# dayae1204/WeCLIP-ViT-CoMer

Hardware: AMD Instinct MI355X
Metric: images/sec (train fwd+bwd) ViT-B/16 512x512 VOC (higher is better)
Workload: dtype f16 MFMA operands / f32 accumulate, f32 residual+softmax+LN, PAR f32 arithmetic on 16-bit fixed-point affinities (precision=fast); 1 GPU; WeCLIP VOC full train step (the reference's model: frozen CLIP ViT-B/16 + adapters + decoder + GradCAM/affinity/PAR pseudo-labels), batch 16/GPU at 512x512, K=2 classes/image (BASELINE configs[2] without the ViT-CoMer inserts, for which the reference has no code); global_batch=16, parallelism=dp1

## Files before the change

include/weclip_hip.h:

```cpp
#ifndef WECLIP_HIP_H
#define WECLIP_HIP_H
#include <stdint.h>
#ifdef __cplusplus
extern "C" {
#endif

int wc_version(void);
const char* wc_last_error(void);
int wc_device_count(void);
int wc_device_arch(int dev, char* buf, int buflen);

void wc_prof_enable(int stride);
void wc_prof_tag(const char* tag);
int wc_prof_report(char* buf, int cap);

int wc_par_affinity(const float* img, float* aff, int B, int H, int W,
                    const int* h_dilations, int n_dil, void* stream);
int wc_par_iterate(const float* aff, const float* masks_in, float* masks_out, int B, int C,
                   int H, int W, const int* h_dilations, int n_dil, void* stream);
int wc_par_forward(const float* img, const float* masks, float* out, float* tmp, float* aff_ws,
                   int B, int C, int H, int W, const int* h_dilations, int n_dil, int num_iter,
                   int group, void* stream);
int wc_par_forward_h(const float* img, const float* masks, float* out, float* tmp, float* aff_ws,
                   int B, int C, int H, int W, const int* h_dilations, int n_dil, int num_iter,
// ... 60 lines not shown
                   int x_rpg, int x_gs, int x_off, int mslice, int bias, float* part, void* stream);
int wc_gemm_km_f16_grouped(const void* dY, long lda, const void* X, long ldx, const void* zeros, int M, int N, int K,
                           int x_rpg, int x_gs, int x_off, int mslice, int bias, float* part, int groups, long gA,
                           long gX, void* stream);
int wc_gemm_km_f16_multi(const int64_t* jobs, int count, const void* zeros, void* stream);
int wc_gemm_km_multi_plan(const int64_t* jobs, int count, int cus, int* launch, int* first, int* pos, int* grids,
                          int* forms, int max_launches, int* nlaunches);
int wc_gemm_km_multi_locate(const int64_t* jobs, int count, int cus, int l, int wg, int* out);
int wc_split_f16(const float* x, void* hi, void* lo, long n, void* stream);

int wc_convert_weights(const int64_t* table, int count, int blocks_per_tensor, void* stream);

int wc_adamw_multi(const int64_t* table, int count, double lr, double beta1, double beta2, double eps,
                   double weight_decay, double bias_correction1, double bias_correction2, int blocks_per_tensor,
                   void* stream);

int wc_sgd_multi(const int64_t* table, int count, double lr, double momentum, double weight_decay, int blocks_per_tensor,
                 void* stream);

int wc_layernorm(const float* x, long ldx, const float* w, const float* b, float eps, float* y32,
                 void* y16, void* y16lo, long rows, int D, void* stream);

int wc_attn_fwd(const void* qkv, void* out, float* out32, float* lse, int B, int L, int H, int DH,
                void* stream);
int wc_attn_mean(const void* qkv, const float* lse, float* mean, int B, int L, int H, int DH,
                 void* stream);

int wc_patchify(const float* img, void* hi, void* lo, int B, int H, int W, int P, void* stream);
int wc_cls_rows(float* x, const float* cls, const float* pos0, int B, int L, int E, void* stream);

int wc_cam_head(const float* x2, const float* lnw, const float* lnb, const float* proj,
                const float* text, const int* text_idx, const int* n_text, const int* pair_img,
                const int* pair_cls, float logit_scale, float* partial, float* probs, float* df,
                int B, int P, int L, int E, int Ed, int Tmax, void* stream);
int wc_lnpost_bwd(const float* df, const float* x2, const float* lnw, float gs, const int* pair_img,
                  float* d32, void* dhi, void* dlo, int P, int L, int E, void* stream);
int wc_ln2_bwd_add(const float* da2, const float* dx2, const float* x1, const float* lnw, float gs,
                   const int* pair_img, void* g16, int P, int L, int E, void* stream);
int wc_attn_bwd_colsum(const void* qkv, const void* dO, const float* o32, const float* lse,
                       const int* pair_img, float* delta, float* u, float* dS0, float* P0, float* c,
                       int P, int L, int H, int DH, void* stream);
int wc_rowvec_matmul(const float* c, const float* W, float* out, float* ws, int P, int N, int E, float scale,
                     void* stream);
int wc_cam_map(const float* a32, const float* w, const int* pair_img, float* cam, int P, int L, int E,
               void* stream);

int wc_aff_weight(const float* const* h_maps, int nmaps, const float* wgt, const float* seg, float* W,
                  int B, int L, void* stream);
int wc_aff_seg_weights(const float* const* h_maps, int nmaps, float* rowsum, float* diff, float* wgt,
                       int B, int L, void* stream);
int wc_matvec(const float* W, const float* X, const float* sin, const float* sout, const float* add,
              float* out, int B, int hw, int K, int transpose, int recip, float alpha, void* stream);
int wc_aff_fused_supported(int hw);
int wc_aff_weight_c1(const float* const* h_maps, int nmaps, const float* wgt, const float* seg, float* W, float* c1,
                     float* ws, int B, int L, void* stream);
int wc_attn_aff_weight(const void* const* h_qkv, const float* const* h_lse, int nmaps, const float* wgt, float* W, float* c1,
                       float* ws, int B, int L, int H, int DH, void* stream);
int wc_aff_sinkhorn_step(const float* W, const float* c, float* r, float* c_next, float* ws, int B, int hw, int last,
                         void* stream);
int wc_aff_tsym_apply(const float* W, const float* r, const float* c, const float* X, float* out, float* y1, float* ws,
                      int B, int hw, int K, void* stream);
int wc_tsym(const float* W, const float* r, const float* c, float* T, int B, int hw, void* stream);
int wc_box_mask(const float* cam, const int* pair_img, const int* pair_slot, float* V, float* mask_out,
                int* boxes, int* nbox, int maxbox, int P, int h, int w, int K, double thr, void* stream);
int wc_cam_upsample(const float* R, const int* nk, float* stats, float* cams, int B, int h, int w, int K,
                    int C, int H, int W, void* stream);

int wc_attn_bwd(const void* qkv, const void* dO, const float* o32, const float* lse, void* qt, void* kt,
                void* dot, float* delta, void* dqkv_hi, void* dqkv_lo, int B, int L, int Lp, int H, int DH,
                void* stream);
int wc_transpose_f16(const void* src, int src_f32, long ld, long sSrc, void* hi, void* lo, long ldo,
                     long oR, int batch, int R, int C, float scale, void* stream);
int wc_colsum(const void* src, int src_f32, long ld, float* part, float* out, long R, int C, float alpha,
              int round16, void* stream);
int wc_layernorm_bwd(const float* dy, const float* x, const float* w, const float* add, float eps,
                     float* dx32, void* dx16, float out_scale, float* part, float* dgb, float alpha,
                     long rows, int D, void* stream);
int wc_layernorm_bwd_h(const void* dy16, const float* x, const float* w, const float* add, float eps,
                       float* dx32, void* dx16, float out_scale, float* part, float* dgb, float alpha,
                       long rows, int D, void* stream);
int wc_layernorm_bwd2_h(const void* dya16, const float* wa, const void* dyb16, const float* wb, const float* x,
                        const float* add, float eps, float* dx32, void* dx16, float out_scale, float* part, float* dgba,
                        float* dgbb, float alpha, long rows, int D, void* stream);
int wc_sigmoid_gram_bwd(const float* dAP, const float* AP, void* hi, void* lo, int B, int n, int ldo,
                        float scale, void* stream);
int wc_colscale_split(const float* x, const float* cs, float* out32, void* hi, void* lo, long rows, int C,
                      int rows_per_batch, float alpha, void* stream);

int wc_msda_fwd(const float* value, const int* h_shapes, int n_levels, const float* loc, const float* attn,
                float* out, int N, int Lq, int M, int D, int P, void* stream);
int wc_msda_fwd_h(const void* value, int value_is_f16, const int* h_shapes, int n_levels, const float* loc,
                  const float* attn, float* out, void* out16, int N, int Lq, int M, int D, int P, void* stream);
int wc_msda_bwd(const float* value, const int* h_shapes, int n_levels, const float* loc, const float* attn,
                const float* gout, float* gvalue, float* gloc, float* gattn, void* gmax, void* ws, int N, int Lq, int M,
                int D, int P, void* stream);
int wc_msda_bwd_h(const void* value, int value_is_f16, const int* h_shapes, int n_levels, const float* loc,
                  const float* attn, const void* gout, int gout_is_f16, float* gvalue, void* gvalue16, float* gloc,
// ... 189 lines not shown
```

weclip-vit-comer_amd/csrc/affinity.hip:

```cpp
#include "common.h"
#include "resample.h"

#define MAXK 4

struct MapPtrs {
    const float* p[12];
};

__global__ __launch_bounds__(256) void aff_weight_kernel(MapPtrs maps, int nmaps, const float* __restrict__ wgt,
                                                          const float* __restrict__ seg, float* __restrict__ W,
                                                          int L) {
    const int hw = L - 1;
    const int j = blockIdx.x * 256 + threadIdx.x, i = blockIdx.y, b = blockIdx.z;
    if (j >= hw) return;
    const long src = (long)b * L * L + (long)(i + 1) * L + (j + 1);
    float v[12];
#pragma unroll
    for (int l = 0; l < 12; ++l) v[l] = l < nmaps ? maps.p[l][src] : 0.f;
    float s = 0.f;
#pragma unroll
    for (int l = 0; l < 12; ++l)
        if (l < nmaps) s = fmaf(wgt[b * nmaps + l], v[l], s);
    const long dst = ((long)b * hw + i) * hw + j;
    if (seg) s *= seg[dst];
// ... 300 lines not shown
    }
}

__global__ __launch_bounds__(256) void aff_colreduce_kernel(const float* __restrict__ colpart, const float* __restrict__ y1,
                                                             const float* __restrict__ c, float* __restrict__ out, int hw,
                                                             int K, int nblk, int mode) {
    const int e = blockIdx.x * 256 + threadIdx.x, b = blockIdx.y;
    if (e >= hw * K) return;
    const float* cp = colpart + (long)b * nblk * hw * K + e;
    const long st = (long)hw * K;
    float s = 0.f;
    int blk = 0;
    for (; blk + 8 <= nblk; blk += 8) {
        float v[8];
#pragma unroll
        for (int u = 0; u < 8; ++u) v[u] = cp[(blk + u) * st];
        s += ((v[0] + v[1]) + (v[2] + v[3])) + ((v[4] + v[5]) + (v[6] + v[7]));
    }
    for (; blk < nblk; ++blk) s += cp[blk * st];
    if (mode == 0) out[(long)b * hw + e] = 1.0f / s;
    else out[(long)b * hw * K + e] = 0.5f * (y1[(long)b * hw * K + e] + c[(long)b * hw + e / K] * s);
}

__global__ __launch_bounds__(256) void tsym_kernel(const float* __restrict__ W, const float* __restrict__ r,
                                                    const float* __restrict__ c, float* __restrict__ T, int hw) {
    const int j = blockIdx.x * 256 + threadIdx.x, i = blockIdx.y, b = blockIdx.z;
    if (j >= hw) return;
    const float* Wb = W + (long)b * hw * hw;
    const float* rb = r + (long)b * hw;
    const float* cb = c + (long)b * hw;
    T[((long)b * hw + i) * hw + j] = 0.5f * (rb[i] * Wb[(long)i * hw + j] * cb[j] + cb[i] * Wb[(long)j * hw + i] * rb[j]);
}

__global__ __launch_bounds__(256) void box_mask_kernel(const float* __restrict__ cam, const int* __restrict__ pair_img,
                                                        const int* __restrict__ pair_slot, float* __restrict__ V,
                                                        float* __restrict__ mask_out, int* __restrict__ boxes,
                                                        int* __restrict__ nbox, int maxbox, int h, int w, int K,
                                                        double thr) {
    extern __shared__ int smi[];
    const int hw = h * w, p = blockIdx.x, tid = threadIdx.x;
    int* lab = smi;
    int* xmin = lab + hw;
    int* xmax = xmin + hw;
    int* ymin = xmax + hw;
    int* ymax = ymin + hw;
    int* roots = ymax + hw;
    int* misc = roots + hw;
    const float* cp = cam + (long)p * hw;
    if (tid == 0) { misc[0] = 0; misc[2] = 0; }
    __syncthreads();
    int mx = 0;
    for (int i = tid; i < hw; i += 256) {
        const int u = (int)(unsigned char)(cp[i] * 255.0f);
        mx = u > mx ? u : mx;
    }
    atomicMax(&misc[0], mx);
    __syncthreads();
    const int theta = (int)(thr * (double)misc[0]);
    for (int i = tid; i < hw; i += 256) {
        const int u = (int)(unsigned char)(cp[i] * 255.0f);
        lab[i] = (u > theta) ? i : -1;
        xmin[i] = w; xmax[i] = -1; ymin[i] = h; ymax[i] = -1;
    }
    __syncthreads();
    for (int it = 0; it < hw + 2; ++it) {
        if (tid == 0) misc[1] = 0;
        __syncthreads();
        int changed = 0;
        for (int i = tid; i < hw; i += 256) {
            int l = lab[i];
            if (l < 0) continue;
// ... 27 lines not shown
        const int y = i / w, x = i - y * w;
        atomicMin(&xmin[l], x); atomicMax(&xmax[l], x);
        atomicMin(&ymin[l], y); atomicMax(&ymax[l], y);
    }
    __syncthreads();
    for (int i = tid; i < hw; i += 256)
        if (lab[i] == i) roots[atomicAdd(&misc[2], 1)] = i;
    __syncthreads();
    const int nroot = misc[2];
    if (boxes) {
        if (tid == 0) nbox[p] = nroot;
        for (int k = tid; k < nroot && k < maxbox; k += 256) {
            const int r = roots[k];
            int* bx = boxes + ((long)p * maxbox + k) * 4;
            bx[0] = xmin[r]; bx[1] = ymin[r];
            bx[2] = (xmax[r] + 1 < w - 1) ? xmax[r] + 1 : w - 1;
            bx[3] = (ymax[r] + 1 < h - 1) ? ymax[r] + 1 : h - 1;
        }
    }
    const int img = pair_img[p], slot = pair_slot[p];
    for (int i = tid; i < hw; i += 256) {
        const int y = i / w, x = i - y * w;
        int inside = 0;
        for (int k = 0; k < nroot && !inside; ++k) {
            const int r = roots[k];
            const int x0 = xmin[r], y0 = ymin[r];
            int x1 = xmax[r] + 1, y1 = ymax[r] + 1;
            x1 = x1 < w - 1 ? x1 : w - 1;
            y1 = y1 < h - 1 ? y1 : h - 1;
            inside = (x >= x0 && x < x1 && y >= y0 && y < y1);
        }
        if (mask_out) mask_out[(long)p * hw + i] = inside ? 1.f : 0.f;
        if (slot >= 0) V[((long)img * hw + i) * K + slot] = inside ? cp[i] : 0.f;
    }
}

__global__ __launch_bounds__(256) void refined_minmax_kernel(const float* __restrict__ R, float* __restrict__ stats,
                                                              int hw, int K) {
    __shared__ float red[16];
    const int k = blockIdx.x, b = blockIdx.y;
    float mn = INFINITY, mx = -INFINITY;
    for (int i = threadIdx.x; i < hw; i += 256) {
        const float v = R[((long)b * hw + i) * K + k];
        mn = fminf(mn, v);
        mx = fmaxf(mx, v);
    }
    mn = block_min(mn, red);
    mx = block_max(mx, red);
    if (threadIdx.x == 0) {
        stats[((long)b * K + k) * 2] = mn;
        stats[((long)b * K + k) * 2 + 1] = mx - mn;
    }
}

__global__ __launch_bounds__(256) void cam_upsample_kernel(const float* __restrict__ R, const float* __restrict__ stats,
                                                            const int* __restrict__ nk, float* __restrict__ cams,
                                                            int h, int w, int K, int C, int H, int W, float sy, float sx) {
    const int x = blockIdx.x * 64 + (threadIdx.x & 63), y = blockIdx.y * 4 + (threadIdx.x >> 6), b = blockIdx.z;
    if (x >= W || y >= H) return;
    int y0, y1, x0, x1;
    float ly, lx;
    wc_bil_src(y, h, sy, y0, y1, ly);
    wc_bil_src(x, w, sx, x0, x1, lx);
    const long HW = (long)H * W;
    const int n = nk[b];
    float best = -INFINITY;
// ... 96 lines not shown
        WC_LAUNCH_CHECK("aff_colreduce_kernel");
    }
    return WC_OK;
}

extern "C" int wc_aff_tsym_apply(const float* W, const float* r, const float* c, const float* X, float* out, float* y1,
                                 float* ws, int B, int hw, int K, void* stream) {
    WC_CHECK_ARG(W && r && c && X && out && y1 && ws && out != X && B > 0 && B <= 65535 && K >= 1 && K <= 4 && aff_fused_ok(hw),
                 "wc_aff_tsym_apply: bad argument (K <= 4)");
    const int nblk = wc_cdiv(hw, AF_RPB);
    hipStream_t st = (hipStream_t)stream;
    dim3 grid(nblk, B);
    const int pr = wc_prof_begin(stream);
    switch (K) {
        case 1: hipLaunchKernelGGL((aff_sweep_kernel<2, 1>), grid, dim3(256), 0, st, W, c, r, X, nullptr, y1, ws, hw); break;
        case 2: hipLaunchKernelGGL((aff_sweep_kernel<2, 2>), grid, dim3(256), 0, st, W, c, r, X, nullptr, y1, ws, hw); break;
        case 3: hipLaunchKernelGGL((aff_sweep_kernel<2, 3>), grid, dim3(256), 0, st, W, c, r, X, nullptr, y1, ws, hw); break;
        default: hipLaunchKernelGGL((aff_sweep_kernel<2, 4>), grid, dim3(256), 0, st, W, c, r, X, nullptr, y1, ws, hw); break;
    }
    wc_prof_end(pr, "aff_sweep_kernel", (double)B * hw * hw * 4.0 * 2, stream);
    WC_LAUNCH_CHECK("aff_sweep_kernel");
    hipLaunchKernelGGL(aff_colreduce_kernel, dim3(wc_cdiv(hw * K, 256), B), dim3(256), 0, st, ws, y1, c, out, hw, K, nblk, 1);
    WC_LAUNCH_CHECK("aff_colreduce_kernel");
    return WC_OK;
}

extern "C" int wc_tsym(const float* W, const float* r, const float* c, float* T, int B, int hw, void* stream) {
    WC_CHECK_ARG(W && r && c && T && B > 0 && hw > 0, "wc_tsym: bad argument");
    hipLaunchKernelGGL(tsym_kernel, dim3(wc_cdiv(hw, 256), hw, B), dim3(256), 0, (hipStream_t)stream, W, r, c, T, hw);
    WC_LAUNCH_CHECK("tsym_kernel");
    return WC_OK;
}

extern "C" int wc_box_mask(const float* cam, const int* pair_img, const int* pair_slot, float* V, float* mask_out,
                           int* boxes, int* nbox, int maxbox, int P, int h, int w, int K, double thr, void* stream) {
    WC_CHECK_ARG(cam && pair_img && pair_slot && V && P > 0 && h > 0 && w > 0 && K > 0, "wc_box_mask: bad argument");
    WC_CHECK_ARG(!boxes || (nbox && maxbox > 0), "wc_box_mask: boxes needs nbox and maxbox");
    const size_t sm = ((size_t)6 * h * w + 4) * sizeof(int);
    WC_CHECK_ARG(sm <= 160 * 1024, "wc_box_mask: CAM grid too large (h*w <= 6800)");
    hipLaunchKernelGGL(box_mask_kernel, dim3(P), dim3(256), sm, (hipStream_t)stream, cam, pair_img, pair_slot, V,
                       mask_out, boxes, nbox, maxbox, h, w, K, thr);
    WC_LAUNCH_CHECK("box_mask_kernel");
    return WC_OK;
}

extern "C" int wc_cam_upsample(const float* R, const int* nk, float* stats, float* cams, int B, int h, int w, int K,
                               int C, int H, int W, void* stream) {
    WC_CHECK_ARG(R && nk && stats && cams && B > 0 && h > 0 && w > 0 && K > 0 && C >= 2 && C <= K + 1 && H > 0 && W > 0,
                 "wc_cam_upsample: bad argument");
    hipStream_t st = (hipStream_t)stream;
    hipLaunchKernelGGL(refined_minmax_kernel, dim3(K, B), dim3(256), 0, st, R, stats, h * w, K);
    WC_LAUNCH_CHECK("refined_minmax_kernel");
    hipLaunchKernelGGL(cam_upsample_kernel, dim3(wc_cdiv(W, 64), wc_cdiv(H, 4), B), dim3(256), 0, st, R, stats, nk,
                       cams, h, w, K, C, H, W, (float)h / H, (float)w / W);
    WC_LAUNCH_CHECK("cam_upsample_kernel");
    return WC_OK;
}
```

weclip-vit-comer_amd/csrc/gradcam.hip:

```cpp
#include "common.h"

typedef _Float16 f16x8 __attribute__((ext_vector_type(8)));
typedef float f32x16 __attribute__((ext_vector_type(16)));

#define LNP_ROWS 16
template <int NV>
__global__ __launch_bounds__(256) void lnpost_pool_kernel(const float* __restrict__ x2,
                                                           const float* __restrict__ w,
                                                           const float* __restrict__ bb, float eps,
                                                           float* __restrict__ partial, int L, int E,
                                                           int nchunk) {
    extern __shared__ float sm[];
    const int b = blockIdx.y, chunk = blockIdx.x, lane = threadIdx.x & 63, wv = threadIdx.x >> 6;
    float acc[NV], wv_[NV], bv[NV];
#pragma unroll
    for (int i = 0; i < NV; ++i) {
        const int e = lane + 64 * i;
        acc[i] = 0.f;
        wv_[i] = e < E ? w[e] : 0.f;
        bv[i] = e < E ? bb[e] : 0.f;
    }
    const int l0 = chunk * LNP_ROWS;
    for (int l = l0 + wv; l < l0 + LNP_ROWS && l < L; l += 4) {
        if (l == 0) continue;
        const float* xr = x2 + ((long)b * L + l) * E;
        float xv[NV];
        float s = 0.f;
#pragma unroll
        for (int i = 0; i < NV; ++i) {
            const int e = lane + 64 * i;
            xv[i] = e < E ? xr[e] : 0.f;
            s += xv[i];
        }
        const float mean = wave_sum(s) / E;
        float q = 0.f;
#pragma unroll
        for (int i = 0; i < NV; ++i) {
            const float d = (lane + 64 * i < E) ? xv[i] - mean : 0.f;
            q += d * d;
        }
        const float rstd = rsqrtf(wave_sum(q) / E + eps);
#pragma unroll
        for (int i = 0; i < NV; ++i)
            if (lane + 64 * i < E) acc[i] += (xv[i] - mean) * rstd * wv_[i] + bv[i];
    }
#pragma unroll
    for (int i = 0; i < NV; ++i)
        if (lane + 64 * i < E) sm[wv * E + lane + 64 * i] = acc[i];
    __syncthreads();
    for (int e = threadIdx.x; e < E; e += 256)
        partial[((long)b * nchunk + chunk) * E + e] = sm[e] + sm[E + e] + sm[2 * E + e] + sm[3 * E + e];
}

__global__ __launch_bounds__(512) void cam_head_kernel(const float* __restrict__ partial,
                                                        const float* __restrict__ proj,
                                                        const float* __restrict__ text,
                                                        const int* __restrict__ text_idx,
                                                        const int* __restrict__ n_text,
                                                        const int* __restrict__ pair_img,
                                                        const int* __restrict__ pair_cls, float logit_scale,
                                                        float* __restrict__ probs, float* __restrict__ df,
                                                        int L, int E, int Ed, int nchunk, int Tmax) {
    extern __shared__ float sm[];
    float* f = sm;
    float* y = f + E;
    float* dy = y + Ed;
    float* lg = dy + Ed;
    float* red = lg + Tmax;
    const int p = blockIdx.x, img = pair_img[p], cls = pair_cls[p], T = n_text[p], tid = threadIdx.x;
    for (int e = tid; e < E; e += 512) {
        const float* pp = partial + (long)img * nchunk * E + e;
        float s[8] = {0.f, 0.f, 0.f, 0.f, 0.f, 0.f, 0.f, 0.f};
        int c = 0;
        for (; c + 8 <= nchunk; c += 8)
#pragma unroll
            for (int u = 0; u < 8; ++u) s[u] += pp[(long)(c + u) * E];
        for (; c < nchunk; ++c) s[0] += pp[(long)c * E];
        f[e] = (((s[0] + s[1]) + (s[2] + s[3])) + ((s[4] + s[5]) + (s[6] + s[7]))) / (L - 1);
    }
    __syncthreads();
    for (int t = tid; t < Ed; t += 512) {
        float s0 = 0.f, s1 = 0.f, s2 = 0.f, s3 = 0.f;
        int e = 0;
        for (; e + 16 <= E; e += 16) {
            float pv[16];
#pragma unroll
            for (int u = 0; u < 16; ++u) pv[u] = proj[(long)(e + u) * Ed + t];
#pragma unroll
            for (int u = 0; u < 16; u += 4) {
                s0 = fmaf(f[e + u], pv[u], s0);
                s1 = fmaf(f[e + u + 1], pv[u + 1], s1);
                s2 = fmaf(f[e + u + 2], pv[u + 2], s2);
                s3 = fmaf(f[e + u + 3], pv[u + 3], s3);
            }
        }
        for (; e < E; ++e) s0 = fmaf(f[e], proj[(long)e * Ed + t], s0);
        y[t] = (s0 + s1) + (s2 + s3);
    }
    __syncthreads();
    float q = 0.f;
    for (int t = tid; t < Ed; t += 512) q += y[t] * y[t];
    const float ynorm = sqrtf(block_sum(q, red));
    __syncthreads();
    for (int t = tid; t < Ed; t += 512) y[t] /= ynorm;
    __syncthreads();
    const int lane = tid & 63, wv = tid >> 6;
    for (int t = wv; t < T; t += 8) {
        const float* tr = text + (long)text_idx[(long)p * Tmax + t] * Ed;
        float s = 0.f;
        for (int k = lane; k < Ed; k += 64) s += y[k] * tr[k];
        s = wave_sum(s);
        if (lane == 0) lg[t] = logit_scale * s;
    }
    __syncthreads();
    float mx = -INFINITY;
    for (int t = 0; t < T; ++t) mx = fmaxf(mx, lg[t]);
    float den = 0.f;
    for (int t = 0; t < T; ++t) den += expf(lg[t] - mx);
    __syncthreads();
    if (tid < T) {
        const float pr = expf(lg[tid] - mx) / den;
        probs[(long)p * Tmax + tid] = pr;
        lg[tid] = pr;
    }
    __syncthreads();
    const float pj = lg[cls];
    for (int k = tid; k < Ed; k += 512) {
        float s = 0.f;
        for (int t = 0; t < T; ++t) {
            const float dl = pj * ((t == cls ? 1.f : 0.f) - lg[t]);
            s = fmaf(dl, text[(long)text_idx[(long)p * Tmax + t] * Ed + k], s);
        }
        dy[k] = logit_scale * s;
    }
    __syncthreads();
    float dot = 0.f;
    for (int k = tid; k < Ed; k += 512) dot += y[k] * dy[k];
    dot = block_sum(dot, red);
    __syncthreads();
    for (int k = tid; k < Ed; k += 512) dy[k] = (dy[k] - y[k] * dot) / ynorm;
    __syncthreads();
    if ((Ed & 3) == 0) {
        const int rsub = lane >> 3, j = lane & 7;
        for (int e0 = wv * 8; e0 < E; e0 += 64) {
            const int e = e0 + rsub;
            float s = 0.f;
            if (e < E) {
                const float* pr = proj + (long)e * Ed;
#pragma unroll 4
                for (int k = 4 * j; k < Ed; k += 32) {
                    const float4 pv = *reinterpret_cast<const float4*>(pr + k);
                    s = fmaf(pv.x, dy[k], s);
                    s = fmaf(pv.y, dy[k + 1], s);
                    s = fmaf(pv.z, dy[k + 2], s);
                    s = fmaf(pv.w, dy[k + 3], s);
                }
            }
            s += __shfl_xor(s, 1, 64);
            s += __shfl_xor(s, 2, 64);
            s += __shfl_xor(s, 4, 64);
            if (j == 0 && e < E) df[(long)p * E + e] = s;
        }
    } else {
        for (int e = tid; e < E; e += 512) {
            const float* pr = proj + (long)e * Ed;
            float s = 0.f;
            for (int k = 0; k < Ed; ++k) s = fmaf(pr[k], dy[k], s);
            df[(long)p * E + e] = s;
        }
    }
}

template <int NV>
__global__ __launch_bounds__(256) void lnpost_bwd_kernel(const float* __restrict__ df,
                                                          const float* __restrict__ x2,
                                                          const float* __restrict__ w, float eps, float gs,
                                                          const int* __restrict__ pair_img,
                                                          float* __restrict__ d32, __half* __restrict__ dhi,
                                                          __half* __restrict__ dlo, int L, int E, long rows) {
    const long row = (long)blockIdx.x * 4 + (threadIdx.x >> 6);
    if (row >= rows) return;
    const int lane = threadIdx.x & 63;
    const int p = row / L, l = row % L;
    const long o = row * E;
    if (l == 0) {
        for (int e = lane; e < E; e += 64) {
            d32[o + e] = 0.f;
            dhi[o + e] = __float2half(0.f);
            if (dlo) dlo[o + e] = __float2half(0.f);
        }
        return;
    }
    const float* xr = x2 + ((long)pair_img[p] * L + l) * E;
    const float* g0 = df + (long)p * E;
    const float invn = 1.0f / (L - 1);
    if constexpr (NV > 0) {
        float xv[NV], gv[NV];
        float s = 0.f;
#pragma unroll
        for (int i = 0; i < NV; ++i) {
            const int e = lane + 64 * i, ec = e < E ? e : 0;
            const float ok = e < E ? 1.f : 0.f;
            xv[i] = xr[ec] * ok;
// ... 405 lines not shown
    const int p = blockIdx.y, img = pair_img[p], lane = threadIdx.x & 63, wv = threadIdx.x >> 6;
    const int l = blockIdx.x * 16 + wv, hw = L - 1;
    if (l >= hw) return;
    const float* ar = a32 + ((long)img * L + l + 1) * E;
    const float* wr = w + (long)p * E;
    float s = 0.f;
    for (int e = lane; e < E; e += 64) s = fmaf(wr[e], ar[e], s);
    s = wave_sum(s);
    if (lane == 0) cam[(long)p * hw + l] = fmaxf(s, 0.f);
}

__global__ __launch_bounds__(1024) void cam_norm_kernel(float* __restrict__ cam, int hw) {
    extern __shared__ float sm[];
    float* cs = sm;
    float* red = cs + hw;
    const int p = blockIdx.x, tid = threadIdx.x;
    for (int l = tid; l < hw; l += 1024) cs[l] = cam[(long)p * hw + l];
    __syncthreads();
#pragma unroll 1
    for (int pass = 0; pass < 2; ++pass) {
        float mn = INFINITY;
        for (int l = tid; l < hw; l += 1024) mn = fminf(mn, cs[l]);
        mn = block_min(mn, red);
        float mx = -INFINITY;
        for (int l = tid; l < hw; l += 1024) mx = fmaxf(mx, cs[l] - mn);
        mx = block_max(mx, red);
        __syncthreads();
        for (int l = tid; l < hw; l += 1024) cs[l] = fmaxf((cs[l] - mn) / (1e-7f + mx), 0.f);
        __syncthreads();
    }
    for (int l = tid; l < hw; l += 1024) cam[(long)p * hw + l] = cs[l];
}

extern "C" int wc_cam_head(const float* x2, const float* lnw, const float* lnb, const float* proj,
                           const float* text, const int* text_idx, const int* n_text, const int* pair_img,
                           const int* pair_cls, float logit_scale, float* partial, float* probs, float* df,
                           int B, int P, int L, int E, int Ed, int Tmax, void* stream) {
    WC_CHECK_ARG(x2 && lnw && lnb && proj && text && text_idx && n_text && pair_img && pair_cls && partial &&
                     probs && df && B > 0 && P > 0 && L > 1 && E > 0 && Ed > 0,
                 "wc_cam_head: bad argument");
    WC_CHECK_ARG(Tmax > 0 && Tmax <= 512 && E <= 4096 && Ed <= 4096, "wc_cam_head: Tmax <= 512, E, Ed <= 4096");
    hipStream_t st = (hipStream_t)stream;
    const int nchunk = wc_cdiv(L, LNP_ROWS);
    WC_CHECK_ARG(E <= 1024, "wc_cam_head: E <= 1024");
    if (E <= 256)
        hipLaunchKernelGGL(lnpost_pool_kernel<4>, dim3(nchunk, B), dim3(256), 4 * E * sizeof(float), st, x2, lnw, lnb,
                           1e-5f, partial, L, E, nchunk);
    else
        hipLaunchKernelGGL(lnpost_pool_kernel<16>, dim3(nchunk, B), dim3(256), 4 * E * sizeof(float), st, x2, lnw, lnb,
                           1e-5f, partial, L, E, nchunk);
    WC_LAUNCH_CHECK("lnpost_pool_kernel");
    const size_t sm = (E + 2 * Ed + Tmax + 16) * sizeof(float);
    hipLaunchKernelGGL(cam_head_kernel, dim3(P), dim3(512), sm, st, partial, proj, text, text_idx, n_text,
                       pair_img, pair_cls, logit_scale, probs, df, L, E, Ed, nchunk, Tmax);
    WC_LAUNCH_CHECK("cam_head_kernel");
    return WC_OK;
}

extern "C" int wc_lnpost_bwd(const float* df, const float* x2, const float* lnw, float gs,
                             const int* pair_img, float* d32, void* dhi, void* dlo, int P, int L, int E,
                             void* stream) {
    WC_CHECK_ARG(df && x2 && lnw && pair_img && d32 && dhi && P > 0 && L > 1 && E > 0,
                 "wc_lnpost_bwd: bad argument");
    const long rows = (long)P * L;
#define LNPOST_BWD(NV_)                                                                                            \
    hipLaunchKernelGGL(lnpost_bwd_kernel<NV_>, dim3(wc_cdiv(rows, 4)), dim3(256), 0, (hipStream_t)stream, df, x2, \
                       lnw, 1e-5f, gs, pair_img, d32, (__half*)dhi, (__half*)dlo, L, E, rows)
    if (E <= 256) LNPOST_BWD(4);
    else if (E <= 768) LNPOST_BWD(12);
    else if (E <= 1024) LNPOST_BWD(16);
    else LNPOST_BWD(0);
#undef LNPOST_BWD
    WC_LAUNCH_CHECK("lnpost_bwd_kernel");
    return WC_OK;
}

extern "C" int wc_ln2_bwd_add(const float* da2, const float* dx2, const float* x1, const float* lnw, float gs,
                              const int* pair_img, void* g16, int P, int L, int E, void* stream) {
    WC_CHECK_ARG(da2 && dx2 && x1 && lnw && pair_img && g16 && P > 0 && L > 0 && E > 0 && gs > 0,
                 "wc_ln2_bwd_add: bad argument");
    const long rows = (long)P * L;
    WC_CHECK_ARG(E <= 1024, "wc_ln2_bwd_add: E <= 1024");
    if (E <= 256)
        hipLaunchKernelGGL(ln2_bwd_add_kernel<4>, dim3(wc_cdiv(rows, 4)), dim3(256), 0, (hipStream_t)stream, da2,
                           dx2, x1, lnw, 1e-5f, 1.0f / gs, pair_img, (__half*)g16, L, E, rows);
    else if (E <= 768)
        hipLaunchKernelGGL(ln2_bwd_add_kernel<12>, dim3(wc_cdiv(rows, 4)), dim3(256), 0, (hipStream_t)stream, da2,
                           dx2, x1, lnw, 1e-5f, 1.0f / gs, pair_img, (__half*)g16, L, E, rows);
    else
// ... 123 lines not shown
```

weclip-vit-comer_amd/gradcam_engine.py:

```python
import torch

from . import _lib as L
from . import ops
from .ops import F16, F32, Split
from .clip import vit_engine as VE

def _logit_scale(clip_model):
    p = clip_model.logit_scale
    key = (p.data_ptr(), p._version)
    cached = getattr(clip_model, "_logit_scale_host", None)
    if cached is None or cached[0] != key:
        cached = (key, float(p.detach().exp().item()))
        clip_model._logit_scale_host = cached
    return cached[1]


GRAD_SCALE = 4096.0


class _BwdPack:

    def __init__(self, blk):
        t = lambda w: ops.split_f16(w.detach().float().t().contiguous())
        self.pjT = t(blk.mlp.c_proj.weight)
        self.fcT = t(blk.mlp.c_fc.weight)
        self.outT = t(blk.attn.out_proj.weight)
        self.w_in = blk.attn.in_proj_weight.detach().float().contiguous()
        self.ln2_w = blk.ln_2.weight.detach().float().contiguous()


class LastLayerState:

    def __init__(self, clip_model, x2, mean, keep, B, Lq):
        self.m, self.x2, self.mean, self.keep, self.B, self.L = clip_model, x2, mean, keep, B, Lq
        blk = clip_model.visual.transformer.resblocks[-1]
        if getattr(blk, "_bwd_pack", None) is None or blk._bwd_pack.w_in.device != x2.device:
            blk._bwd_pack = _BwdPack(blk)
        self.bw = blk._bwd_pack
        self.blk = blk

    def _head(self, text_hat, text_idx, n_text, pair_img, pair_cls, Tmax):
        v = self.m.visual
        B, Lq = self.B, self.L
        E, Ed = v.proj.shape
        P = pair_img.numel()
        dev = self.x2.device
        nchunk = (Lq + 15) // 16
        partial = torch.empty(B * nchunk * E, device=dev, dtype=F32)
        probs = torch.zeros(P, Tmax, device=dev, dtype=F32)
        df = torch.empty(P, E, device=dev, dtype=F32)
        L.lib().wc_cam_head(L.ptr(self.x2, F32), L.ptr(v.ln_post.weight.detach().float(), F32),
                            L.ptr(v.ln_post.bias.detach().float(), F32),
                            L.ptr(v.proj.detach().float().contiguous(), F32), L.ptr(text_hat, F32),
                            L.ptr(text_idx, torch.int32), L.ptr(n_text, torch.int32),
                            L.ptr(pair_img, torch.int32), L.ptr(pair_cls, torch.int32),
                            _logit_scale(self.m), L.ptr(partial), L.ptr(probs),
                            L.ptr(df), B, P, Lq, E, Ed, Tmax, L.stream())
        return probs, df

    def class_probs(self, text):
        dev = self.x2.device
        T = text.shape[0]
        that = (text / text.norm(dim=1, keepdim=True)).contiguous()
        idx = torch.arange(T, dtype=torch.int32, device=dev).repeat(self.B, 1).contiguous()
        nt = torch.full((self.B,), T, dtype=torch.int32, device=dev)
        img = torch.arange(self.B, dtype=torch.int32, device=dev)
        cls = torch.zeros(self.B, dtype=torch.int32, device=dev)
        probs, _ = self._head(that, idx, nt, img, cls, T)
        return probs

    def grad_cam(self, text_hat, text_idx, n_text, pair_img, pair_cls, Tmax):
        lib = L.lib()
        k, bw = self.keep, self.bw
        B, Lq = self.B, self.L
        E = self.x2.shape[1]
        H = self.blk.attn.num_heads
        DH = E // H
        P = pair_img.numel()
        M = P * Lq
        dev = self.x2.device
        st = L.stream
        probs, df = self._head(text_hat, text_idx, n_text, pair_img, pair_cls, Tmax)
        v = self.m.visual
        dx2 = torch.empty(M, E, device=dev, dtype=F32)
        from . import config
        ex = config.exact()
        dx2s = Split(torch.empty(M, E, device=dev, dtype=F16), torch.empty(M, E, device=dev, dtype=F16) if ex else None)
        lib.wc_lnpost_bwd(L.ptr(df), L.ptr(self.x2), L.ptr(v.ln_post.weight.detach().float(), F32),
                          GRAD_SCALE, L.ptr(pair_img), L.ptr(dx2), L.ptr(dx2s.hi), L.ptr(dx2s.lo), P, Lq, E,
                          st())
# ... 29 lines not shown
```

Measured before the change: 1314 images/sec.

## Parallelize CAM head and box-mask kernels across more blocks and threads

The CAM head is split into three kernels: a per-image projection spread over many blocks, a per-pair softmax/gradient kernel, and a df kernel tiled over rows of the projection. This replaces the single block per pair that recomputed the full projection serially. The box-mask connected-component kernel now runs with up to 1024 threads per block instead of 256 and caches each thread's cam value. The old single-block paths remain as _single entry points. These are small pseudo-label stages, so the gain in end-to-end throughput is likely modest, and the split adds launches and intermediate buffers.

```diff
diff --git a/include/weclip_hip.h b/include/weclip_hip.h
--- a/include/weclip_hip.h
+++ b/include/weclip_hip.h
@@ -116,7 +116,11 @@
 int wc_cam_head(const float* x2, const float* lnw, const float* lnb, const float* proj,
                 const float* text, const int* text_idx, const int* n_text, const int* pair_img,
                 const int* pair_cls, float logit_scale, float* partial, float* probs, float* df,
-                int B, int P, int L, int E, int Ed, int Tmax, void* stream);
+                float* y, float* dy, int B, int P, int L, int E, int Ed, int Tmax, void* stream);
+int wc_cam_head_single(const float* x2, const float* lnw, const float* lnb, const float* proj,
+                       const float* text, const int* text_idx, const int* n_text, const int* pair_img,
+                       const int* pair_cls, float logit_scale, float* partial, float* probs, float* df,
+                       float* y, float* dy, int B, int P, int L, int E, int Ed, int Tmax, void* stream);
 int wc_lnpost_bwd(const float* df, const float* x2, const float* lnw, float gs, const int* pair_img,
                   float* d32, void* dhi, void* dlo, int P, int L, int E, void* stream);
 int wc_ln2_bwd_add(const float* da2, const float* dx2, const float* x1, const float* lnw, float gs,
@@ -147,6 +151,8 @@
 int wc_tsym(const float* W, const float* r, const float* c, float* T, int B, int hw, void* stream);
 int wc_box_mask(const float* cam, const int* pair_img, const int* pair_slot, float* V, float* mask_out,
                 int* boxes, int* nbox, int maxbox, int P, int h, int w, int K, double thr, void* stream);
+int wc_box_mask_single(const float* cam, const int* pair_img, const int* pair_slot, float* V, float* mask_out,
+                       int* boxes, int* nbox, int maxbox, int P, int h, int w, int K, double thr, void* stream);
 int wc_cam_upsample(const float* R, const int* nk, float* stats, float* cams, int B, int h, int w, int K,
                     int C, int H, int W, void* stream);
 
diff --git a/weclip-vit-comer_amd/csrc/affinity.hip b/weclip-vit-comer_amd/csrc/affinity.hip
--- a/weclip-vit-comer_amd/csrc/affinity.hip
+++ b/weclip-vit-comer_amd/csrc/affinity.hip
@@ -356,11 +356,11 @@
     T[((long)b * hw + i) * hw + j] = 0.5f * (rb[i] * Wb[(long)i * hw + j] * cb[j] + cb[i] * Wb[(long)j * hw + i] * rb[j]);
 }
 
-__global__ __launch_bounds__(256) void box_mask_kernel(const float* __restrict__ cam, const int* __restrict__ pair_img,
-                                                        const int* __restrict__ pair_slot, float* __restrict__ V,
-                                                        float* __restrict__ mask_out, int* __restrict__ boxes,
-                                                        int* __restrict__ nbox, int maxbox, int h, int w, int K,
-                                                        double thr) {
+__global__ __launch_bounds__(256) void box_mask_single_kernel(const float* __restrict__ cam, const int* __restrict__ pair_img,
+                                                               const int* __restrict__ pair_slot, float* __restrict__ V,
+                                                               float* __restrict__ mask_out, int* __restrict__ boxes,
+                                                               int* __restrict__ nbox, int maxbox, int h, int w, int K,
+                                                               double thr) {
     extern __shared__ int smi[];
     const int hw = h * w, p = blockIdx.x, tid = threadIdx.x;
     int* lab = smi;
@@ -454,6 +454,130 @@
         }
         if (mask_out) mask_out[(long)p * hw + i] = inside ? 1.f : 0.f;
         if (slot >= 0) V[((long)img * hw + i) * K + slot] = inside ? cp[i] : 0.f;
+    }
+}
+
+__global__ __launch_bounds__(1024) void box_mask_kernel(const float* __restrict__ cam, const int* __restrict__ pair_img,
+                                                         const int* __restrict__ pair_slot, float* __restrict__ V,
+                                                         float* __restrict__ mask_out, int* __restrict__ boxes,
+                                                         int* __restrict__ nbox, int maxbox, int h, int w, int K,
+                                                         double thr) {
+    extern __shared__ int smi[];
+    const int hw = h * w, p = blockIdx.x, tid = threadIdx.x, nthr = blockDim.x;
+    int* lab = smi;
+    int* xmin = lab + hw;
+    int* xmax = xmin + hw;
+    int* ymin = xmax + hw;
+    int* ymax = ymin + hw;
+    int* roots = ymax + hw;
+    int* misc = roots + hw;
+    const float* cp = cam + (long)p * hw;
+    const float c0 = tid < hw ? cp[tid] : 0.f;
+    auto camv = [&](int i) { return i == tid ? c0 : cp[i]; };
+    if (tid < 4) misc[tid] = 0;
+    __syncthreads();
+    int mx = 0;
+    for (int i = tid; i < hw; i += nthr) {
+        const int u = (int)(unsigned char)(camv(i) * 255.0f);
+        mx = u > mx ? u : mx;
+    }
+#pragma unroll
+    for (int o = 32; o > 0; o >>= 1) {
+        const int v = __shfl_xor(mx, o, 64);
+        mx = v > mx ? v : mx;
+    }
+    if ((tid & 63) == 0) atomicMax(&misc[0], mx);
+    __syncthreads();
+    const int theta = (int)(thr * (double)misc[0]);
+    for (int i = tid; i < hw; i += nthr) {
+        const int u = (int)(unsigned char)(camv(i) * 255.0f);
+        lab[i] = (u > theta) ? i : -1;
+        xmin[i] = w; xmax[i] = -1; ymin[i] = h; ymax[i] = -1;
+    }
+    __syncthreads();
+    for (int it = 0; it < hw + 2; ++it) {
+        int* flag = misc + 1 + 2 * (it & 1);
+        int changed = 0;
+        for (int i = tid; i < hw; i += nthr) {
+            const int l = lab[i];
+            if (l < 0) continue;
+            const int y = i / w, x = i - y * w;
+            const int r0 = (y > 0 ? y - 1 : y) * w, r1 = y * w, r2 = (y < h - 1 ? y + 1 : y) * w;
+            const int xa = x > 0 ? x - 1 : x, xb = x < w - 1 ? x + 1 : x;
+            const unsigned n0 = lab[r0 + xa], n1 = lab[r0 + x], n2 = lab[r0 + xb], n3 = lab[r1 + xa], n4 = lab[r1 + xb],
+                           n5 = lab[r2 + xa], n6 = lab[r2 + x], n7 = lab[r2 + xb];
+            const unsigned best = min(min(min(n0, n1), min(n2, n3)), min(min(n4, n5), min(n6, n7)));
+            if (best < (unsigned)l) { lab[i] = (int)best; changed = 1; }
+        }
+        if (changed) *flag = 1;
+        if (tid == 0) misc[1 + 2 * ((it + 1) & 1)] = 0;
+        __syncthreads();
+        if (*flag == 0) break;
+        for (int i = tid; i < hw; i += nthr) {
+            const int l = lab[i];
+            if (l >= 0) {
+                const int ll = lab[l];
+                if (ll < l) lab[i] = ll;
+            }
+        }
+        __syncthreads();
+    }
+    for (int i = tid; i < hw; i += nthr) {
+        const int l = lab[i];
+        if (l < 0) continue;
+        const int y = i / w, x = i - y * w;
+        if (x == 0 || lab[i - 1] < 0) atomicMin(&xmin[l], x);
+        if (x == w - 1 || lab[i + 1] < 0) atomicMax(&xmax[l], x);
+        if (y == 0 || lab[i - w] < 0) atomicMin(&ymin[l], y);
+        if (y == h - 1 || lab[i + w] < 0) atomicMax(&ymax[l], y);
+        if (l == i) roots[atomicAdd(&misc[2], 1)] = i;
+    }
+    __syncthreads();
+    const int nroot = misc[2];
+    if (boxes) {
+        if (tid == 0) nbox[p] = nroot;
+        for (int k = tid; k < nroot && k < maxbox; k += nthr) {
+            const int r = roots[k];
+            int* bx = boxes + ((long)p * maxbox + k) * 4;
+            bx[0] = xmin[r]; bx[1] = ymin[r];
+            bx[2] = (xmax[r] + 1 < w - 1) ? xmax[r] + 1 : w - 1;
+            bx[3] = (ymax[r] + 1 < h - 1) ? ymax[r] + 1 : h - 1;
+        }
+    }
+    int* cnt = lab;
+    for (int i = tid; i < hw; i += nthr) cnt[i] = 0;
+    __syncthreads();
+    for (int k = tid; k < nroot; k += nthr) {
+        const int r = roots[k];
+        const int x0 = xmin[r], y0 = ymin[r];
+        int x1 = xmax[r] + 1, y1 = ymax[r] + 1;
+        x1 = x1 < w - 1 ? x1 : w - 1;
+        y1 = y1 < h - 1 ? y1 : h - 1;
+        if (x1 > x0 && y1 > y0) {
+            atomicAdd(&cnt[y0 * w + x0], 1);
+            atomicAdd(&cnt[y0 * w + x1], -1);
+            atomicAdd(&cnt[y1 * w + x0], -1);
+            atomicAdd(&cnt[y1 * w + x1], 1);
+        }
+    }
+    __syncthreads();
+    for (int x = tid; x < w; x += nthr) {
+        int s = 0;
+#pragma unroll 8
+        for (int y = 0; y < h; ++y) { s += cnt[y * w + x]; cnt[y * w + x] = s; }
+    }
+    __syncthreads();
+    for (int y = tid; y < h; y += nthr) {
+        int s = 0;
+#pragma unroll 8
+        for (int x = 0; x < w; ++x) { s += cnt[y * w + x]; cnt[y * w + x] = s; }
+    }
+    __syncthreads();
+    const int img = pair_img[p], slot = pair_slot[p];
+    for (int i = tid; i < hw; i += nthr) {
+        const bool inside = cnt[i] > 0;
+        if (mask_out) mask_out[(long)p * hw + i] = inside ? 1.f : 0.f;
+        if (slot >= 0) V[((long)img * hw + i) * K + slot] = inside ? camv(i) : 0.f;
     }
 }
 
@@ -616,16 +740,33 @@
     return WC_OK;
 }
 
-extern "C" int wc_box_mask(const float* cam, const int* pair_img, const int* pair_slot, float* V, float* mask_out,
-                           int* boxes, int* nbox, int maxbox, int P, int h, int w, int K, double thr, void* stream) {
+static int box_mask_launch(const float* cam, const int* pair_img, const int* pair_slot, float* V, float* mask_out, int* boxes,
+                           int* nbox, int maxbox, int P, int h, int w, int K, double thr, void* stream, bool wide) {
     WC_CHECK_ARG(cam && pair_img && pair_slot && V && P > 0 && h > 0 && w > 0 && K > 0, "wc_box_mask: bad argument");
     WC_CHECK_ARG(!boxes || (nbox && maxbox > 0), "wc_box_mask: boxes needs nbox and maxbox");
     const size_t sm = ((size_t)6 * h * w + 4) * sizeof(int);
     WC_CHECK_ARG(sm <= 160 * 1024, "wc_box_mask: CAM grid too large (h*w <= 6800)");
-    hipLaunchKernelGGL(box_mask_kernel, dim3(P), dim3(256), sm, (hipStream_t)stream, cam, pair_img, pair_slot, V,
-                       mask_out, boxes, nbox, maxbox, h, w, K, thr);
-    WC_LAUNCH_CHECK("box_mask_kernel");
-    return WC_OK;
+    if (wide) {
+        const int nthr = h * w >= 1024 ? 1024 : (h * w + 63) / 64 * 64;
+        hipLaunchKernelGGL(box_mask_kernel, dim3(P), dim3(nthr), sm, (hipStream_t)stream, cam, pair_img, pair_slot, V,
+                           mask_out, boxes, nbox, maxbox, h, w, K, thr);
+        WC_LAUNCH_CHECK("box_mask_kernel");
+    } else {
+        hipLaunchKernelGGL(box_mask_single_kernel, dim3(P), dim3(256), sm, (hipStream_t)stream, cam, pair_img, pair_slot, V,
+                           mask_out, boxes, nbox, maxbox, h, w, K, thr);
+        WC_LAUNCH_CHECK("box_mask_single_kernel");
+    }
+    return WC_OK;
+}
+
+extern "C" int wc_box_mask(const float* cam, const int* pair_img, const int* pair_slot, float* V, float* mask_out,
+                           int* boxes, int* nbox, int maxbox, int P, int h, int w, int K, double thr, void* stream) {
+    return box_mask_launch(cam, pair_img, pair_slot, V, mask_out, boxes, nbox, maxbox, P, h, w, K, thr, stream, true);
+}
+
+extern "C" int wc_box_mask_single(const float* cam, const int* pair_img, const int* pair_slot, float* V, float* mask_out,
+                                  int* boxes, int* nbox, int maxbox, int P, int h, int w, int K, double thr, void* stream) {
+    return box_mask_launch(cam, pair_img, pair_slot, V, mask_out, boxes, nbox, maxbox, P, h, w, K, thr, stream, false);
 }
 
 extern "C" int wc_cam_upsample(const float* R, const int* nk, float* stats, float* cams, int B, int h, int w, int K,
diff --git a/weclip-vit-comer_amd/csrc/gradcam.hip b/weclip-vit-comer_amd/csrc/gradcam.hip
--- a/weclip-vit-comer_amd/csrc/gradcam.hip
+++ b/weclip-vit-comer_amd/csrc/gradcam.hip
@@ -50,6 +50,129 @@
     __syncthreads();
     for (int e = threadIdx.x; e < E; e += 256)
         partial[((long)b * nchunk + chunk) * E + e] = sm[e] + sm[E + e] + sm[2 * E + e] + sm[3 * E + e];
+}
+
+template <int NQ>
+__device__ __forceinline__ void cam_head_pool(const float* __restrict__ partial, float* f, int img, int L, int E, int nchunk) {
+    const int nthr = blockDim.x;
+    for (int e0 = threadIdx.x; e0 < E; e0 += NQ * nthr) {
+        const float* pp[NQ];
+        float s[NQ][8];
+#pragma unroll
+        for (int q = 0; q < NQ; ++q) {
+            const int e = e0 + q * nthr;
+            pp[q] = partial + (long)img * nchunk * E + (e < E ? e : E - 1);
+#pragma unroll
+            for (int u = 0; u < 8; ++u) s[q][u] = 0.f;
+        }
+        int c = 0;
+        for (; c + 8 <= nchunk; c += 8)
+#pragma unroll
+            for (int q = 0; q < NQ; ++q)
+#pragma unroll
+                for (int u = 0; u < 8; ++u) s[q][u] += pp[q][(long)(c + u) * E];
+        for (; c < nchunk; ++c)
+#pragma unroll
+            for (int q = 0; q < NQ; ++q) s[q][0] += pp[q][(long)c * E];
+#pragma unroll
+        for (int q = 0; q < NQ; ++q)
+            if (e0 + q * nthr < E)
+                f[e0 + q * nthr] = (((s[q][0] + s[q][1]) + (s[q][2] + s[q][3])) + ((s[q][4] + s[q][5]) + (s[q][6] + s[q][7]))) / (L - 1);
+    }
+}
+
+__device__ __forceinline__ void cam_head_pair_part(float* y, float* dy, float* lg, float* red, const float* __restrict__ text,
+                                                   const int* __restrict__ text_idx, int p, int T, int cls, float logit_scale,
+                                                   float* __restrict__ probs, int Ed, int Tmax) {
+    const int tid = threadIdx.x;
+    float q = 0.f;
+    for (int t = tid; t < Ed; t += 512) q += y[t] * y[t];
+    const float ynorm = sqrtf(block_sum(q, red));
+    __syncthreads();
+    for (int t = tid; t < Ed; t += 512) y[t] /= ynorm;
+    __syncthreads();
+    const int lane = tid & 63, wv = tid >> 6;
+    for (int t = wv; t < T; t += 8) {
+        const float* tr = text + (long)text_idx[(long)p * Tmax + t] * Ed;
+        float s = 0.f;
+        for (int k = lane; k < Ed; k += 64) s += y[k] * tr[k];
+        s = wave_sum(s);
+        if (lane == 0) lg[t] = logit_scale * s;
+    }
+    __syncthreads();
+    float mx = -INFINITY;
+    for (int t = 0; t < T; ++t) mx = fmaxf(mx, lg[t]);
+    float den = 0.f;
+    for (int t = 0; t < T; ++t) den += expf(lg[t] - mx);
+    __syncthreads();
+    if (tid < T) {
+        const float pr = expf(lg[tid] - mx) / den;
+        probs[(long)p * Tmax + tid] = pr;
+        lg[tid] = pr;
+    }
+    __syncthreads();
+    const float pj = lg[cls];
+    for (int k = tid; k < Ed; k += 512) {
+        float s = 0.f;
+        for (int t0 = 0; t0 < T; t0 += 8) {
+            float tv[8];
+#pragma unroll
+            for (int u = 0; u < 8; ++u) {
+                const int t = t0 + u < T ? t0 + u : T - 1;
+                tv[u] = text[(long)text_idx[(long)p * Tmax + t] * Ed + k];
+            }
+#pragma unroll
+            for (int u = 0; u < 8; ++u) {
+                const int t = t0 + u;
+                if (t < T) {
+                    const float dl = pj * ((t == cls ? 1.f : 0.f) - lg[t]);
+                    s = fmaf(dl, tv[u], s);
+                }
+            }
+        }
+        dy[k] = logit_scale * s;
+    }
+    __syncthreads();
+    float dot = 0.f;
+    for (int k = tid; k < Ed; k += 512) dot += y[k] * dy[k];
+    dot = block_sum(dot, red);
+    __syncthreads();
+    for (int k = tid; k < Ed; k += 512) dy[k] = (dy[k] - y[k] * dot) / ynorm;
+    __syncthreads();
+}
+
+__device__ __forceinline__ void cam_head_df_rows(const float* __restrict__ proj, const float* dy, float* __restrict__ dfp, int Ed,
+                                                 int ebeg, int eend) {
+    const int tid = threadIdx.x, lane = tid & 63, wv = tid >> 6;
+    if ((Ed & 3) == 0) {
+        const int rsub = lane >> 3, j = lane & 7;
+        for (int e0 = ebeg + wv * 8; e0 < eend; e0 += 64) {
+            const int e = e0 + rsub;
+            float s = 0.f;
+            if (e < eend) {
+                const float* pr = proj + (long)e * Ed;
+#pragma unroll 4
+                for (int k = 4 * j; k < Ed; k += 32) {
+                    const float4 pv = *reinterpret_cast<const float4*>(pr + k);
+                    s = fmaf(pv.x, dy[k], s);
+                    s = fmaf(pv.y, dy[k + 1], s);
+                    s = fmaf(pv.z, dy[k + 2], s);
+                    s = fmaf(pv.w, dy[k + 3], s);
+                }
+            }
+            s += __shfl_xor(s, 1, 64);
+            s += __shfl_xor(s, 2, 64);
+            s += __shfl_xor(s, 4, 64);
+            if (j == 0 && e < eend) dfp[e] = s;
+        }
+    } else {
+        for (int e = ebeg + tid; e < eend; e += 512) {
+            const float* pr = proj + (long)e * Ed;
+            float s = 0.f;
+            for (int k = 0; k < Ed; ++k) s = fmaf(pr[k], dy[k], s);
+            dfp[e] = s;
+        }
+    }
 }
 
 __global__ __launch_bounds__(512) void cam_head_kernel(const float* __restrict__ partial,
@@ -68,16 +191,7 @@
     float* lg = dy + Ed;
     float* red = lg + Tmax;
     const int p = blockIdx.x, img = pair_img[p], cls = pair_cls[p], T = n_text[p], tid = threadIdx.x;
-    for (int e = tid; e < E; e += 512) {
-        const float* pp = partial + (long)img * nchunk * E + e;
-        float s[8] = {0.f, 0.f, 0.f, 0.f, 0.f, 0.f, 0.f, 0.f};
-        int c = 0;
-        for (; c + 8 <= nchunk; c += 8)
-#pragma unroll
-            for (int u = 0; u < 8; ++u) s[u] += pp[(long)(c + u) * E];
-        for (; c < nchunk; ++c) s[0] += pp[(long)c * E];
-        f[e] = (((s[0] + s[1]) + (s[2] + s[3])) + ((s[4] + s[5]) + (s[6] + s[7]))) / (L - 1);
-    }
+    cam_head_pool<1>(partial, f, img, L, E, nchunk);
     __syncthreads();
     for (int t = tid; t < Ed; t += 512) {
         float s0 = 0.f, s1 = 0.f, s2 = 0.f, s3 = 0.f;
@@ -98,77 +212,62 @@
         y[t] = (s0 + s1) + (s2 + s3);
     }
     __syncthreads();
-    float q = 0.f;
-    for (int t = tid; t < Ed; t += 512) q += y[t] * y[t];
-    const float ynorm = sqrtf(block_sum(q, red));
-    __syncthreads();
-    for (int t = tid; t < Ed; t += 512) y[t] /= ynorm;
-    __syncthreads();
-    const int lane = tid & 63, wv = tid >> 6;
-    for (int t = wv; t < T; t += 8) {
-        const float* tr = text + (long)text_idx[(long)p * Tmax + t] * Ed;
-        float s = 0.f;
-        for (int k = lane; k < Ed; k += 64) s += y[k] * tr[k];
-        s = wave_sum(s);
-        if (lane == 0) lg[t] = logit_scale * s;
-    }
-    __syncthreads();
-    float mx = -INFINITY;
-    for (int t = 0; t < T; ++t) mx = fmaxf(mx, lg[t]);
-    float den = 0.f;
-    for (int t = 0; t < T; ++t) den += expf(lg[t] - mx);
-    __syncthreads();
-    if (tid < T) {
-        const float pr = expf(lg[tid] - mx) / den;
-        probs[(long)p * Tmax + tid] = pr;
-        lg[tid] = pr;
-    }
-    __syncthreads();
-    const float pj = lg[cls];
-    for (int k = tid; k < Ed; k += 512) {
-        float s = 0.f;
-        for (int t = 0; t < T; ++t) {
-            const float dl = pj * ((t == cls ? 1.f : 0.f) - lg[t]);
-            s = fmaf(dl, text[(long)text_idx[(long)p * Tmax + t] * Ed + k], s);
-        }
-        dy[k] = logit_scale * s;
-    }
-    __syncthreads();
-    float dot = 0.f;
-    for (int k = tid; k < Ed; k += 512) dot += y[k] * dy[k];
-    dot = block_sum(dot, red);
-    __syncthreads();
-    for (int k = tid; k < Ed; k += 512) dy[k] = (dy[k] - y[k] * dot) / ynorm;
-    __syncthreads();
-    if ((Ed & 3) == 0) {
-        const int rsub = lane >> 3, j = lane & 7;
-        for (int e0 = wv * 8; e0 < E; e0 += 64) {
-            const int e = e0 + rsub;
-            float s = 0.f;
-            if (e < E) {
-                const float* pr = proj + (long)e * Ed;
-#pragma unroll 4
-                for (int k = 4 * j; k < Ed; k += 32) {
-                    const float4 pv = *reinterpret_cast<const float4*>(pr + k);
-                    s = fmaf(pv.x, dy[k], s);
-                    s = fmaf(pv.y, dy[k + 1], s);
-                    s = fmaf(pv.z, dy[k + 2], s);
-                    s = fmaf(pv.w, dy[k + 3], s);
-                }
-            }
-            s += __shfl_xor(s, 1, 64);
-            s += __shfl_xor(s, 2, 64);
-            s += __shfl_xor(s, 4, 64);
-            if (j == 0 && e < E) df[(long)p * E + e] = s;
-        }
-    } else {
-        for (int e = tid; e < E; e += 512) {
-            const float* pr = proj + (long)e * Ed;
-            float s = 0.f;
-            for (int k = 0; k < Ed; ++k) s = fmaf(pr[k], dy[k], s);
-            df[(long)p * E + e] = s;
-        }
-    }
+    cam_head_pair_part(y, dy, lg, red, text, text_idx, p, T, cls, logit_scale, probs, Ed, Tmax);
+    cam_head_df_rows(proj, dy, df + (long)p * E, Ed, 0, E);
+}
+
+__global__ __launch_bounds__(256) void cam_head_y_kernel(const float* __restrict__ partial, const float* __restrict__ proj,
+                                                          float* __restrict__ yg, int L, int E, int Ed, int nchunk) {
+    extern __shared__ float sm[];
+    float* f = sm;
+    float* sp = f + E;
+    const int img = blockIdx.y, lane = threadIdx.x & 63, j = threadIdx.x >> 6;
+    cam_head_pool<4>(partial, f, img, L, E, nchunk);
+    __syncthreads();
+    const int t = blockIdx.x * 64 + lane;
+    const float* pc = proj + (t < Ed ? t : Ed - 1);
+    const int E16 = E & ~15;
+    float s = 0.f;
+    int e = j;
+    for (; e + 124 < E16; e += 128) {
+        float pv[32];
+#pragma unroll
+        for (int u = 0; u < 32; ++u) pv[u] = pc[(long)(e + 4 * u) * Ed];
+#pragma unroll
+        for (int u = 0; u < 32; ++u) s = fmaf(f[e + 4 * u], pv[u], s);
+    }
+    for (; e < E16; e += 4) s = fmaf(f[e], pc[(long)e * Ed], s);
+    if (j == 0)
+        for (e = E16; e < E; ++e) s = fmaf(f[e], pc[(long)e * Ed], s);
+    sp[j * 64 + lane] = s;
+    __syncthreads();
+    if (j == 0 && t < Ed) yg[(long)img * Ed + t] = (sp[lane] + sp[64 + lane]) + (sp[128 + lane] + sp[192 + lane]);
+}
+
+__global__ __launch_bounds__(512) void cam_head_pair_kernel(const float* __restrict__ yg, const float* __restrict__ text,
+                                                             const int* __restrict__ text_idx, const int* __restrict__ n_text,
+                                                             const int* __restrict__ pair_img, const int* __restrict__ pair_cls,
+                                                             float logit_scale, float* __restrict__ probs,
+                                                             float* __restrict__ dyg, int Ed, int Tmax) {
+    extern __shared__ float sm[];
+    float* y = sm;
+    float* dy = y + Ed;
+    float* lg = dy + Ed;
+    float* red = lg + Tmax;
+    const int p = blockIdx.x, img = pair_img[p], tid = threadIdx.x;
+    for (int t = tid; t < Ed; t += 512) y[t] = yg[(long)img * Ed + t];
+    __syncthreads();
+    cam_head_pair_part(y, dy, lg, red, text, text_idx, p, n_text[p], pair_cls[p], logit_scale, probs, Ed, Tmax);
+    for (int k = tid; k < Ed; k += 512) dyg[(long)p * Ed + k] = dy[k];
+}
+
+__global__ __launch_bounds__(512) void cam_head_df_kernel(const float* __restrict__ proj, const float* __restrict__ dyg,
+                                                           float* __restrict__ df, int E, int Ed) {
+    extern __shared__ float sm[];
+    const int p = blockIdx.y, ebeg = blockIdx.x * 64;
+    for (int k = threadIdx.x; k < Ed; k += 512) sm[k] = dyg[(long)p * Ed + k];
+    __syncthreads();
+    cam_head_df_rows(proj, sm, df + (long)p * E, Ed, ebeg, ebeg + 64 < E ? ebeg + 64 : E);
 }
 
 template <int NV>
@@ -640,17 +739,18 @@
     for (int l = tid; l < hw; l += 1024) cam[(long)p * hw + l] = cs[l];
 }
 
-extern "C" int wc_cam_head(const float* x2, const float* lnw, const float* lnb, const float* proj,
-                           const float* text, const int* text_idx, const int* n_text, const int* pair_img,
-                           const int* pair_cls, float logit_scale, float* partial, float* probs, float* df,
-                           int B, int P, int L, int E, int Ed, int Tmax, void* stream) {
+static int cam_head_launch(const float* x2, const float* lnw, const float* lnb, const float* proj, const float* text,
+                           const int* text_idx, const int* n_text, const int* pair_img, const int* pair_cls,
+                           float logit_scale, float* partial, float* probs, float* df, float* y, float* dy, int B, int P,
+                           int L, int E, int Ed, int Tmax, void* stream, bool wide) {
     WC_CHECK_ARG(x2 && lnw && lnb && proj && text && text_idx && n_text && pair_img && pair_cls && partial &&
-                     probs && df && B > 0 && P > 0 && L > 1 && E > 0 && Ed > 0,
+                     probs && df && y && dy && B > 0 && P > 0 && L > 1 && E > 0 && Ed > 0,
                  "wc_cam_head: bad argument");
     WC_CHECK_ARG(Tmax > 0 && Tmax <= 512 && E <= 4096 && Ed <= 4096, "wc_cam_head: Tmax <= 512, E, Ed <= 4096");
     hipStream_t st = (hipStream_t)stream;
     const int nchunk = wc_cdiv(L, LNP_ROWS);
     WC_CHECK_ARG(E <= 1024, "wc_cam_head: E <= 1024");
+    WC_CHECK_ARG(B <= 65535 && P <= 65535, "wc_cam_head: too many images/pairs for one launch");
     if (E <= 256)
         hipLaunchKernelGGL(lnpost_pool_kernel<4>, dim3(nchunk, B), dim3(256), 4 * E * sizeof(float), st, x2, lnw, lnb,
                            1e-5f, partial, L, E, nchunk);
@@ -658,11 +758,38 @@
         hipLaunchKernelGGL(lnpost_pool_kernel<16>, dim3(nchunk, B), dim3(256), 4 * E * sizeof(float), st, x2, lnw, lnb,
                            1e-5f, partial, L, E, nchunk);
     WC_LAUNCH_CHECK("lnpost_pool_kernel");
-    const size_t sm = (E + 2 * Ed + Tmax + 16) * sizeof(float);
-    hipLaunchKernelGGL(cam_head_kernel, dim3(P), dim3(512), sm, st, partial, proj, text, text_idx, n_text,
-                       pair_img, pair_cls, logit_scale, probs, df, L, E, Ed, nchunk, Tmax);
-    WC_LAUNCH_CHECK("cam_head_kernel");
+    if (!wide) {
+        const size_t sm = (E + 2 * Ed + Tmax + 16) * sizeof(float);
+        hipLaunchKernelGGL(cam_head_kernel, dim3(P), dim3(512), sm, st, partial, proj, text, text_idx, n_text,
+                           pair_img, pair_cls, logit_scale, probs, df, L, E, Ed, nchunk, Tmax);
+        WC_LAUNCH_CHECK("cam_head_kernel");
+        return WC_OK;
+    }
+    hipLaunchKernelGGL(cam_head_y_kernel, dim3(wc_cdiv(Ed, 64), B), dim3(256), (E + 256) * sizeof(float), st, partial, proj, y,
+                       L, E, Ed, nchunk);
+    WC_LAUNCH_CHECK("cam_head_y_kernel");
+    hipLaunchKernelGGL(cam_head_pair_kernel, dim3(P), dim3(512), (2 * Ed + Tmax + 16) * sizeof(float), st, y, text, text_idx,
+                       n_text, pair_img, pair_cls, logit_scale, probs, dy, Ed, Tmax);
+    WC_LAUNCH_CHECK("cam_head_pair_kernel");
+    hipLaunchKernelGGL(cam_head_df_kernel, dim3(wc_cdiv(E, 64), P), dim3(512), Ed * sizeof(float), st, proj, dy, df, E, Ed);
+    WC_LAUNCH_CHECK("cam_head_df_kernel");
     return WC_OK;
+}
+
+extern "C" int wc_cam_head(const float* x2, const float* lnw, const float* lnb, const float* proj,
+                           const float* text, const int* text_idx, const int* n_text, const int* pair_img,
+                           const int* pair_cls, float logit_scale, float* partial, float* probs, float* df,
+                           float* y, float* dy, int B, int P, int L, int E, int Ed, int Tmax, void* stream) {
+    return cam_head_launch(x2, lnw, lnb, proj, text, text_idx, n_text, pair_img, pair_cls, logit_scale, partial, probs, df,
+                           y, dy, B, P, L, E, Ed, Tmax, stream, true);
+}
+
+extern "C" int wc_cam_head_single(const float* x2, const float* lnw, const float* lnb, const float* proj,
+                                  const float* text, const int* text_idx, const int* n_text, const int* pair_img,
+                                  const int* pair_cls, float logit_scale, float* partial, float* probs, float* df,
+                                  float* y, float* dy, int B, int P, int L, int E, int Ed, int Tmax, void* stream) {
+    return cam_head_launch(x2, lnw, lnb, proj, text, text_idx, n_text, pair_img, pair_cls, logit_scale, partial, probs, df,
+                           y, dy, B, P, L, E, Ed, Tmax, stream, false);
 }
 
 extern "C" int wc_lnpost_bwd(const float* df, const float* x2, const float* lnw, float gs,
diff --git a/weclip-vit-comer_amd/gradcam_engine.py b/weclip-vit-comer_amd/gradcam_engine.py
--- a/weclip-vit-comer_amd/gradcam_engine.py
+++ b/weclip-vit-comer_amd/gradcam_engine.py
@@ -49,13 +49,15 @@
         partial = torch.empty(B * nchunk * E, device=dev, dtype=F32)
         probs = torch.zeros(P, Tmax, device=dev, dtype=F32)
         df = torch.empty(P, E, device=dev, dtype=F32)
+        y = torch.empty(B, Ed, device=dev, dtype=F32)
+        dy = torch.empty(P, Ed, device=dev, dtype=F32)
         L.lib().wc_cam_head(L.ptr(self.x2, F32), L.ptr(v.ln_post.weight.detach().float(), F32),
                             L.ptr(v.ln_post.bias.detach().float(), F32),
                             L.ptr(v.proj.detach().float().contiguous(), F32), L.ptr(text_hat, F32),
                             L.ptr(text_idx, torch.int32), L.ptr(n_text, torch.int32),
                             L.ptr(pair_img, torch.int32), L.ptr(pair_cls, torch.int32),
                             _logit_scale(self.m), L.ptr(partial), L.ptr(probs),
-                            L.ptr(df), B, P, Lq, E, Ed, Tmax, L.stream())
+                            L.ptr(df), L.ptr(y), L.ptr(dy), B, P, Lq, E, Ed, Tmax, L.stream())
         return probs, df
 
     def class_probs(self, text):
```

Result: faster. 1337 images/sec, median of 6 (+1.7%).
